# luigifreda/plvs

Hardware: AMD Instinct MI355X
Metric: Mvoxels/sec TSDF integrate (chisel 5 cm / 5 m, 640x480 RGB-D) (higher is better)
Workload: dtype f32; 1 GPU; configs[2] stand-in, STREAMING: see DESIGN.md 4.1 / 4.6; mode=order-free (fixed-point sums; sdf / weight within tolerance), longest_voxel_run=25008, parallelism=chunk-hash shard x1

## Files before the change

### plvs_amd/csrc/tsdf_chisel.hip

```cpp
#include "tsdf_chisel_handle.hpp"
#include "tsdf_chisel_halo.hpp"
#include "tsdf_chisel_ordered.hpp"
#include "tsdf_chisel_order_free.hpp"
#include "tsdf_chisel_carve.hpp"
#include "tsdf_chisel_shard.hpp"
#include "tsdf_chisel_deform.hpp"
#include "tsdf_chisel_scan.hpp"

namespace {

__global__ void pool_init(float* __restrict__ sdf, size_t n) {
  const size_t i = (size_t)blockIdx.x * blockDim.x + threadIdx.x;
  const size_t stride = (size_t)gridDim.x * blockDim.x;
  for (size_t j = i; j < n; j += stride) sdf[j] = 99999.0f;
}

__global__ void selftest_sort_fill(uint32_t* __restrict__ keys, uint32_t* __restrict__ v32, unsigned long long* __restrict__ v64,
                                   uint32_t n, int bits, uint32_t seed) {
  const uint32_t i = blockIdx.x * blockDim.x + threadIdx.x;
  if (i >= n) return;
  uint32_t x = (i + 1u) * 2654435761u + seed;
  x ^= x << 13; x ^= x >> 17; x ^= x << 5;
  x ^= x << 13; x ^= x >> 17; x ^= x << 5;
  keys[i] = bits >= 32 ? x : (x & ((1u << bits) - 1u));
// ... 227 lines not shown
  (void)hipFree(h->weight);
  (void)hipFree(h->kfid);
  (void)hipFree(h->rgbw);
  (void)hipFree(h->d_ctr);
  if (h->h_ctr) (void)hipHostFree(h->h_ctr);
  (void)hipFree(h->d_wctr);
  if (h->h_wctr) (void)hipHostFree(h->h_wctr);
  if (h->h_seq) (void)hipHostFree(h->h_seq);
  if (h->h_offsets) (void)hipHostFree(h->h_offsets);
  (void)hipFree(h->gdir.keys);
  (void)hipFree(h->gdir.slots);
  (void)hipFree(h->miss_keys);
  (void)hipFree(h->miss_ids);
  (void)hipFree(h->miss_count);
  (void)hipFree(h->xdir.keys);
  (void)hipFree(h->xdir.slots);
  (void)hipFree(h->xdir.slot_ids);
  (void)hipFree(h->d_xcount);
  (void)hipFree(h->x_sat);
  if (h->h_sh_counts) (void)hipHostFree(h->h_sh_counts);
  if (h->h_sh_ctl) (void)hipHostFree(h->h_sh_ctl);
  if (h->h_sh_off) (void)hipHostFree(h->h_sh_off);
  h->q_xyz.release(); h->q_rgb.release(); h->q_kfid.release();
  h->w_rec.release(); h->w_seg.release(); h->w_sorted_seg.release(); h->w_chunk_nseg.release();
  h->w_chunk_off.release(); h->w_chunk_fill.release(); h->w_active_off.release(); h->w_masks.release();
  h->w_dummy.release(); h->w_runkey.release(); h->w_run_cnt.release(); h->w_run_off.release(); h->w_val0.release();
  h->w_val1.release(); h->w_seg_cnt.release(); h->w_tile_visits.release(); h->w_deferred.release(); h->w_part_off.release(); h->w_multi_idx.release();
  h->pa_wuu.release(); h->pa_w.release(); h->pa_last.release(); h->pa_cnt.release(); h->pa_done.release();
  h->sh_nrec.release(); h->sh_owner.release(); h->halo_row.release();
  h->sh_ctl.release(); h->sh_seg_reg.release(); h->sh_rec_reg.release(); h->sh_src_off.release(); h->sh_slot_owner.release(); h->sh_run_ctr.release(); h->sh_vkey.release(); h->sh_sat.release(); h->sh_wait.release(); h->sh_run_first.release();
  if (h->ev_fork) (void)hipEventDestroy(h->ev_fork);
  if (h->ev_join) (void)hipEventDestroy(h->ev_join);
  if (h->ev_seg) (void)hipEventDestroy(h->ev_seg);
  if (h->ev_zero) (void)hipEventDestroy(h->ev_zero);
  h->w_rseg.release(); h->w_rpre.release(); h->w_run_matrix.release(); h->w_active_idx.release(); h->w_item_base.release();
  h->w_item_cnt.release(); h->w_item_part0.release(); h->w_part_item.release(); h->w_phist.release();
  h->w_row_heads.release(); h->w_row_tot.release();
  if (h->side) (void)hipStreamDestroy(h->side);
  for (int i = 0; i <= kNumStages; ++i)
    if (h->ev[i]) (void)hipEventDestroy(h->ev[i]);
  h->counts.release();
  h->rec.release(); h->rec_t.release(); h->recc_t.release();
  h->dkey0.release(); h->dkey1.release(); h->didx0.release(); h->didx1.release();
  h->last_pt.release(); h->run_cnt.release(); h->run_dst.release();
  h->tile_first.release(); h->block_first.release(); h->tile_state.release();
  h->heads.release(); h->updated.release(); h->scratch.release(); h->poses.release();
  h->offsets.release(); h->st_xyz.release(); h->st_Twc.release(); h->st_nrm.release(); h->st_rgb.release();
// ... 505 lines not shown
```

### plvs_amd/csrc/tsdf_chisel_handle.hpp

```cpp
#pragma once
#include <vector>

#include "common.hpp"
#include "device_utils.hpp"
#include "tsdf_chisel_core.hpp"
#include "tsdf_directory.hpp"
#include "tsdf_chisel_view.hpp"
#include "tsdf_walk.hpp"
#include "tsdf_walk_plan.hpp"

using namespace plvs;
using namespace plvs::chisel;
using namespace plvs::tsdf;

namespace {

constexpr int kNumStages = 6;
const char* const kStageNames[kNumStages] = {"ray_count", "scan", "ray_tiles", "sort_runs",
                                             "gather_runs", "chain_runs"};
constexpr int kWalkStages = 4;
const char* const kWalkStageNames[kWalkStages] = {"walk_tiles", "sort_segments", "apply_chunks", "fold_colours"};

struct Counters {
  uint32_t total_visits;
// ... 72 lines not shown
  unsigned long long* miss_keys = nullptr;
  int32_t* miss_ids = nullptr;
  uint32_t* miss_count = nullptr;
  uint32_t miss_cap = 0, miss_mask = 0;
  DevBuf<int32_t> offsets;
  DevBuf<float> st_xyz, st_Twc, st_nrm;
  DevBuf<uint8_t> st_rgb;
  DevBuf<uint32_t> st_kfid;
  DevBuf<uint32_t> st_pos, st_scan, st_off;
  plvs_tsdf_stats stats{};
  uint32_t last_updated = 0;
  DevBuf<float> q_xyz;
  DevBuf<uint8_t> q_rgb;
  DevBuf<uint32_t> q_kfid;
  std::vector<int32_t> q_offsets;
  std::vector<float> q_Twc;
  bool q_kfid_given = false;
  WalkCounters* d_wctr = nullptr;
  WalkCounters* h_wctr = nullptr;
  uint32_t* h_seq = nullptr;
  uint32_t seq_next = 0;
  double wait_ema_us[3][3] = {{0.0, 0.0, 0.0}, {0.0, 0.0, 0.0}, {0.0, 0.0, 0.0}};
  DevBuf<uint4> w_rec, w_seg, w_sorted_seg;
  DevBuf<uint4> w_rseg, w_rpre;
  DevBuf<uint32_t> w_run_matrix, w_active_idx, w_item_base, w_item_cnt, w_item_part0, w_part_item, w_phist, w_row_heads, w_row_tot;
  hipEvent_t ev_zero = nullptr;
  hipEvent_t ev_seg = nullptr;
  int last_chain = 0;
  bool last_chain_skipped = false;
  DevBuf<uint32_t> w_chunk_nseg, w_chunk_off, w_chunk_fill, w_active_off, w_masks, w_dummy, w_seg_cnt, w_tile_visits, w_deferred;
  DevBuf<uint32_t> w_part_off, w_multi_idx;
  DevBuf<long long> pa_wuu;
  DevBuf<unsigned long long> pa_w;
  DevBuf<uint32_t> pa_last, pa_cnt, pa_done;
  uint32_t multi_cap = 0;
  uint32_t part_segs = kPartSegs, part_min = kPartMin;
  plvs::tsdf::WalkHistory walk;
  DevBuf<uint32_t> w_runkey, w_run_cnt, w_run_off, w_val0, w_val1;
  int32_t* h_offsets = nullptr;
  size_t h_offsets_cap = 0;
  uint32_t run_r1_log2 = 11;
  float scale_u = 1.f, scale_w = 1.f;
  int stage_set = 0;
  Directory xdir{};
  int32_t* d_xcount = nullptr;
  uint32_t* x_sat = nullptr;
// ... 131 lines not shown
```

### plvs_amd/csrc/tsdf_chisel_order_free.hpp

```cpp
#pragma once
#include "tsdf_chisel_handle.hpp"

namespace {

__global__ void walk_prologue(const float* __restrict__ Twc, int nclouds, Pose* __restrict__ poses,
                              const int32_t* __restrict__ host_offsets, int32_t* __restrict__ offsets,
                              WalkCounters* __restrict__ wctr, Counters* __restrict__ ctr, uint32_t* __restrict__ chunk_nseg,
                              int nseg, int ntile_first = 0) {
  const int i0 = blockIdx.x * blockDim.x + threadIdx.x, stride = gridDim.x * blockDim.x;
  for (int c = i0; c < nclouds; c += stride) make_pose(Twc + 12 * c, &poses[c]);
  for (int c = i0; c < 2 * (nclouds + 1) + ntile_first; c += stride) offsets[c] = host_offsets[c];
  for (int k = i0; k < nseg; k += stride) chunk_nseg[k] = 0u;
  uint32_t* w = reinterpret_cast<uint32_t*>(wctr);
  for (int k = i0; k < (int)(2 * sizeof(WalkCounters) / sizeof(uint32_t)); k += stride) w[k] = 0u;
  if (i0 == 0) {
    ctr->total_visits = 0;
    ctr->err = 0;
    ctr->num_heads = 0;
    ctr->num_updated = 0;
    ctr->max_run = 0;
    ctr->num_desc = 0;
  }
}

// ... 54 lines not shown
  PLVS_HIP_TRY(hipMemset(h->pa_cnt.p, 0, nv * sizeof(uint32_t)));
  PLVS_HIP_TRY(hipMemset(h->pa_done.p, 0, nd * sizeof(uint32_t)));
  h->multi_cap = chunks;
  return PLVS_OK;
}

static int reserve_chunk_tables(plvs_tsdf_chisel* h, size_t chunks, uint32_t part_chunks) {
  PLVS_HIP_TRY(h->w_chunk_nseg.reserve(chunks));
  PLVS_HIP_TRY(h->w_chunk_off.reserve(chunks + 1));
  PLVS_HIP_TRY(h->w_chunk_fill.reserve(chunks));
  PLVS_HIP_TRY(h->w_active_off.reserve(chunks + 1));
  PLVS_HIP_TRY(h->updated.reserve(chunks + 1));
  PLVS_HIP_TRY(h->w_part_off.reserve(chunks + 1));
  PLVS_HIP_TRY(h->w_multi_idx.reserve(chunks + 1));
  return ensure_part_acc(h, part_chunks);
}


struct SegSrc {
  size_t slots;
  uint32_t seg_cap, ntiles;
  const uint32_t* seg_cnt;
};
template <bool kScatter, int kSpan = kSegSpan>
static void launch_seg_pass(plvs_tsdf_chisel* h, const SegSrc& src, hipStream_t q) {
  hipLaunchKernelGGL((seg_pass<kScatter, kSpan>), dim3(ceil_div(src.slots, kSpan)), dim3(256), 0, q, h->w_seg.p, src.seg_cap,
                     src.ntiles, src.seg_cnt, h->w_chunk_nseg.p, h->w_chunk_off.p, h->w_chunk_fill.p, h->w_sorted_seg.p,
                     h->d_wctr);
}

struct SegScan {
  const int32_t* num_chunks;
  int chunk_cap;
  const uint32_t *tile_visits, *run_cnt;
  uint32_t ntiles;
  uint32_t* active_idx;
};
static void launch_seg_scan(plvs_tsdf_chisel* h, const SegScan& a, hipStream_t q) {
  hipLaunchKernelGGL(seg_scan, dim3(1), dim3(1024), 0, q, h->w_chunk_nseg.p, h->w_chunk_off.p, h->w_chunk_fill.p, h->updated.p,
                     h->w_active_off.p, h->d_wctr, a.num_chunks, a.chunk_cap, a.tile_visits, a.run_cnt, a.ntiles,
                     h->w_part_off.p, h->w_multi_idx.p, h->multi_cap, h->part_segs, h->part_min, a.active_idx);
}

static void sort_segments(plvs_tsdf_chisel* h, const SegSrc& src, const SegScan& scan, hipStream_t q) {
  launch_seg_pass<false>(h, src, q);
  launch_seg_scan(h, scan, q);
  launch_seg_pass<true>(h, src, q);
}

template <bool kWide, bool kEmit>
static void launch_apply(plvs_tsdf_chisel* h, const uint4* rec, const uint32_t* d_kfid, const EmitOut& emit, uint32_t last_shift,
// ... 1 lines not shown
  hipLaunchKernelGGL((apply_chunks<kWide, kEmit>), dim3(4096), dim3(kApplyThreads), 0, q, h->w_sorted_seg.p, h->updated.p,
                     h->w_active_off.p, h->w_part_off.p, h->w_multi_idx.p, h->part_segs,
                     PartAcc{h->pa_wuu.p, h->pa_w.p, h->pa_last.p, h->pa_cnt.p, h->pa_done.p}, rec,
                     kEmit ? 0.0 : 1.0 / (double)h->scale_u, kEmit ? 0.0 : 1.0 / (double)h->scale_w, d_kfid,
                     kEmit ? (float*)nullptr : h->sdf, kEmit ? (float*)nullptr : h->weight, kEmit ? (uint32_t*)nullptr : h->kfid,
                     h->d_wctr, emit, last_shift);
}

struct WalkScratch {
  size_t rec_own, seg_own, rec_spill, seg_spill;
};
static WalkScratch walk_scratch(const plvs_tsdf_chisel* h, uint32_t ntiles) {
  WalkScratch w;
  w.rec_own = (size_t)ntiles * kRecStride;
  w.seg_own = (size_t)ntiles * kWalkChunks;
  w.rec_spill = std::max<size_t>(h->w_rec.cap > w.rec_own ? h->w_rec.cap - w.rec_own : 0, (size_t)1 << 16);
  w.seg_spill = std::max<size_t>(h->w_seg.cap / 2 > w.seg_own ? h->w_seg.cap / 2 - w.seg_own : 0, (size_t)1 << 12);
  return w;
}
static int reserve_walk_scratch(plvs_tsdf_chisel* h, uint32_t ntiles, const WalkScratch& w) {
  if (h->w_rec.cap < w.rec_own + w.rec_spill) PLVS_HIP_TRY(h->w_rec.reserve(2 * w.rec_own + w.rec_spill));
  if (h->w_seg.cap < 2 * (w.seg_own + w.seg_spill)) PLVS_HIP_TRY(h->w_seg.reserve(2 * (2 * w.seg_own + w.seg_spill)));
  PLVS_HIP_TRY(h->w_sorted_seg.reserve(h->w_seg.cap));
  const size_t run_slots = (size_t)ntiles << h->run_r1_log2;
  if (h->w_runkey.cap < run_slots) {
    PLVS_HIP_TRY(h->w_runkey.reserve(2 * run_slots));
    PLVS_HIP_TRY(h->w_masks.reserve(2 * run_slots * kMaskWords));
  }
  PLVS_HIP_TRY(h->w_masks.reserve(run_slots * kMaskWords));
  return PLVS_OK;
}
static AccOut walk_out(const plvs_tsdf_chisel* h, const WalkScratch& w, uint32_t* chunk_nseg) {
  return AccOut{h->w_rec.p, (uint32_t)std::min<size_t>(w.rec_own + w.rec_spill, 0xFFFFFFFFu), h->w_seg.p,
                (uint32_t)std::min<size_t>(w.seg_own + w.seg_spill, 0xFFFFFFFFu), h->w_seg_cnt.p, h->w_tile_visits.p, chunk_nseg};
}
static bool grow_walk_scratch(plvs_tsdf_chisel* h, uint32_t ntiles, WalkScratch& w) {
  w.rec_spill = std::max<size_t>(w.rec_spill, (size_t)h->h_wctr->rec_top * 2);
  w.seg_spill = std::max<size_t>(w.seg_spill, (size_t)h->h_wctr->seg_top * 2);
  while ((1u << h->run_r1_log2) < h->h_wctr->run_need) ++h->run_r1_log2;
  return ((size_t)ntiles << h->run_r1_log2) < 0xFFFFFFFFull;
}


struct WalkCall {
  const float* d_xyz;
  const uint8_t* d_rgb;
  const uint32_t* d_kfid;
  int n, nclouds;
  uint32_t ntiles;
  int max_chunks;
  const GridSrc* gsrc;
  const GridSrc* d_grid;
  size_t seg_slots;
  AccOut out;
  RunOut runs;
  const uint32_t* last_count;
  uint32_t collect_seq;
// ... 12 lines not shown
}

static void launch_walk_passes(plvs_tsdf_chisel* h, const WalkPlan& plan, const WalkCall& c, hipStream_t s) {
  for (int i = 0; i < plan.npasses; ++i) {
    const WalkPass& pass = plan.pass[i];
    if (pass.entries == kPlanSmallClass) launch_walk_fast<kFastEntriesSmall>(h, c, pass, s);
    else if (pass.entries == kFastEntries) launch_walk_fast<kFastEntries>(h, c, pass, s);
    else launch_walk_fast<kFastEntriesBig>(h, c, pass, s);
  }
  hipLaunchKernelGGL((walk_tiles<true, true>), dim3(kDeferGrid), dim3(kWalkRays), 0, s, h->P, h->scale_u, h->scale_w, c.d_xyz,
                     c.n, h->offsets.p, c.nclouds, h->poses.p, h->dir, &h->d_ctr->num_chunks, h->d_wctr, h->rgbw,
                     (const uint32_t*)nullptr, c.out, c.runs, TileMap{1u, 0u, 1u}, c.ntiles,
                     (const uint32_t*)(h->w_deferred.p + (size_t)plan.last_list * c.ntiles), c.last_count, kRecStride,
                     plan.pieces, c.d_grid);
}

static int segments_and_apply(plvs_tsdf_chisel* h, const WalkPlan& plan, const WalkCall& c, hipStream_t q) {
  launch_seg_scan(h, SegScan{&h->d_ctr->num_chunks, c.max_chunks, h->w_tile_visits.p, h->w_run_cnt.p, c.ntiles,
                             plan.collect_ready ? h->w_active_idx.p : nullptr}, q);
  if (plan.collect_ready) {
    const bool queued = plan.chain == kChainCollected;
    PLVS_HIP_TRY(hipStreamWaitEvent(q, h->ev_zero, 0));
    hipLaunchKernelGGL(runs_count, dim3(plan.collect_blocks), dim3(kSegSpan), 0, q, h->w_seg.p, h->w_rseg.p, c.ntiles, h->w_seg_cnt.p,
                       h->w_active_idx.p, plan.collect_rows, plan.collect_blocks, h->w_run_matrix.p, h->w_rpre.p, h->d_wctr, c.last_count);
    hipLaunchKernelGGL(runs_rowscan, dim3(std::min<uint32_t>(ceil_div(plan.collect_rows, 4), 1024u)), dim3(256), 0, q,
                       h->w_run_matrix.p, plan.collect_rows, plan.collect_blocks, h->d_wctr, h->w_item_cnt.p);
    hipLaunchKernelGGL(rows_place, dim3(1), dim3(1024), 0, q, h->w_item_cnt.p, plan.collect_rows, plan.collect_bound,
                       (uint32_t)std::min<size_t>(plan.parts_cap, 0xFFFFFFFFu), h->d_wctr,
                       h->w_item_base.p, h->w_item_part0.p, h->w_part_item.p, reinterpret_cast<const uint32_t*>(h->d_ctr),
                       reinterpret_cast<uint32_t*>(h->h_wctr), reinterpret_cast<uint32_t*>(h->h_ctr),
                       (uint32_t)(sizeof(Counters) / sizeof(uint32_t)), queued ? h->h_seq : (uint32_t*)nullptr,
                       queued ? c.collect_seq : 0u);
    PLVS_HIP_TRY(hipEventRecord(h->ev_seg, q));
  }
  const SegSrc src{c.seg_slots, c.out.seg_cap, c.ntiles, h->w_seg_cnt.p};
  if (plan.size_class == 2) launch_seg_pass<true, kSegSpanLong>(h, src, q);
  else launch_seg_pass<true>(h, src, q);
  PLVS_HIP_TRY(stage_mark(h, 2, q));
  launch_apply<false, false>(h, h->w_rec.p, c.d_kfid, EmitOut{}, c.gsrc ? c.gsrc->key_bits : 0u, q);
  PLVS_KERNEL_CHECK();
  PLVS_HIP_TRY(stage_mark(h, 3, q));
  return PLVS_OK;
}

static int launch_fold(plvs_tsdf_chisel* h, const WalkCall& c, uint32_t D, const uint32_t* skeys, const uint32_t* sval,
                       const uint32_t* skip, hipStream_t q) {
  const RunSrc rsrc{h->w_masks.p, (uint32_t)kMaskWords, h->run_r1_log2, TileMap{1u, 0u}, h->offsets.p, c.nclouds,
                    reinterpret_cast<const uint32_t*>(h->offsets.p) + 2 * ((size_t)c.nclouds + 1)};
  const auto kernel = c.gsrc ? fold_colours_masks<true> : fold_colours_masks<false>;
  hipLaunchKernelGGL(kernel, dim3(std::min<size_t>(ceil_div(D, kFoldWaves), 8192)), dim3(64 * kFoldWaves), 0, q, skeys, sval,
                     &h->d_wctr[1].num_desc, rsrc, h->heads.p, c.d_rgb, h->rgbw, &h->d_wctr[1].num_heads, (uint32_t*)nullptr,
                     (uint32_t*)nullptr, skip, c.gsrc ? *c.gsrc : GridSrc{});
  PLVS_KERNEL_CHECK();
  return PLVS_OK;
}

template <int BITS>
static void launch_sort_medium(plvs_tsdf_chisel* h, uint32_t ntiles, int passes, const RunGuard* guard, hipStream_t q) {
  hipLaunchKernelGGL(sort_runs_medium<BITS>, dim3(1), dim3(1024), 0, q, h->w_runkey.p, h->w_run_cnt.p, ntiles, h->run_r1_log2,
                     h->d_wctr + 1, h->dkey0.p, h->w_val0.p, h->dkey1.p, h->w_val1.p, h->w_run_off.p, h->heads.p, passes,
// ... 267 lines not shown
```

### plvs_amd/csrc/tsdf_walk.hpp

```cpp
#pragma once
#include <hip/hip_runtime.h>

#include <cstdint>

#include "tsdf_chisel_core.hpp"
#include "tsdf_directory.hpp"
#include "tsdf_tiles.hpp"
#include "tsdf_walk_table.hpp"

namespace {

using namespace plvs::chisel;
using plvs::tsdf::cloud_of;
using plvs::tsdf::tile_span;
using plvs::tsdf::tile_span_tables;
using plvs::tsdf::TileSpan;
using plvs::tsdf::kCoordBias;
using plvs::tsdf::kErrCoordRange;
using plvs::tsdf::kErrDirectoryMiss;
using plvs::tsdf::kErrPoolFull;
using plvs::tsdf::home_bucket;
using plvs::tsdf::next_bucket;

constexpr int kWalkRays = 512;
// ... 468 lines not shown
__device__ __forceinline__ DirPeek dir_peek(const Directory& d, int cx, int cy, int cz) {
  DirPeek p;
  p.key = kEmptyKey;
  p.slot = -1;
  if (!pack_block(cx, cy, cz, &p.want)) {
    p.want = 0;
    return p;
  }
  const uint32_t h = dir_hash(cx, cy, cz, d.mask);
  p.key = d.keys[h];
  p.slot = d.slots[h];
  return p;
}
__device__ __forceinline__ int dir_peek_slot(const DirPeek& p) { return (p.key == p.want && p.slot >= 0) ? p.slot : -1; }

struct AccOut {
  uint4* rec;
  uint32_t rec_cap;
  uint4* seg;
  uint32_t seg_cap;
  uint32_t* seg_cnt;
  uint32_t* tile_visits;
  uint32_t* chunk_nseg;
};
struct RunOut {
  uint32_t* dkey;
  uint32_t* masks;
  uint32_t* run_cnt;
  uint32_t r1_log2;
  uint4* rseg;
};

constexpr int kMaskCap = kWalkEntries / 4;

__device__ __forceinline__ uint4 pack_suboffsets(const uint32_t* o) {
  return make_uint4(o[0] | (o[1] << 16), o[2] | (o[3] << 16), o[4] | (o[5] << 16), o[6] | (o[7] << 16));
}

struct TileMap {
  uint32_t stride, first;
  uint32_t tables;
  __device__ __host__ uint32_t tile_of(uint32_t local) const { return local * stride + first; }
};

template <bool kAcc, bool kRuns>
__global__ __launch_bounds__(kWalkRays, kWalkEntries > 2048 ? 2 : (kWalkEntries > 1024 ? 4 : 6)) void walk_tiles(
// ... 229 lines not shown
      if (ci[k] >= 0) {
        slot_of[k] = S.cslot[ci[k]];
        if (slot_of[k] >= 0) rank[k] = atomicAdd(&S.ccnt[ci[k] * kSlabs + (int)(vid / kSlabVox)], 1u);
      } else {
        int cx, cy, cz;
        chunk_of_code(chunk_code(ekey[k]), fox, foy, foz, &cx, &cy, &cz);
        slot_of[k] = dir_find_or_insert(dir, cx, cy, cz, num_chunks, &ctr->err);
      }
      if (slot_of[k] >= 0) {
        vkey[k] = (uint32_t)slot_of[k] * (uint32_t)kChunkVox + vid;
        const bool cold = sat ? ((sat[vkey[k] >> 5] >> (vkey[k] & 31u)) & 1u) == 0u : (rgbw[vkey[k]] >> 24) < 254u;
        if (kRuns && cold) {
          need |= 1u << k;
          ++nneed;
          multi = multi || (uint32_t)(ewc[k] >> 32) > 1u;
        }
      }
    }
    const bool any_multi = __syncthreads_or(multi ? 1 : 0) != 0;
    WALK_PROF(5);
    if (kAcc) {
      const bool own_region = flushes == 0;
      uint32_t rbase = tile * rec_stride;
      if (own_region || tid < 64) {
        const int cl = lane;
        uint32_t sub[kSlabs], c = 0;
#pragma unroll
        for (int s = 0; s < kSlabs; ++s) {
          sub[s] = c;
          c += S.ccnt[cl * kSlabs + s];
        }
        uint32_t inc = c, sinc = c ? 1u : 0u;
#pragma unroll
        for (int off = 1; off < 64; off <<= 1) {
          const uint32_t up = (uint32_t)__shfl_up((int)inc, off), sup = (uint32_t)__shfl_up((int)sinc, off);
          if (lane >= off) { inc += up; sinc += sup; }
        }
        const uint32_t tot = (uint32_t)__shfl((int)inc, 63), stot = (uint32_t)__shfl((int)sinc, 63);
        uint32_t sbase = tile * (uint32_t)kWalkChunks;
        if (!own_region) {
          if (tid == 0 && tot) {
            rbase = ntiles * rec_stride + atomicAdd(&ctr->rec_top, tot);
            sbase = ntiles * (uint32_t)kWalkChunks + atomicAdd(&ctr->seg_top, stot);
            if (rbase + tot > out.rec_cap || sbase + stot > out.seg_cap) atomicOr(&ctr->err, kErrScratch);
          }
          rbase = (uint32_t)__shfl((int)rbase, 0);
          sbase = (uint32_t)__shfl((int)sbase, 0);
          if (tid == 0) S.rbase = rbase;
        } else if (tid == 0) {
          out.seg_cnt[tile] = stot;
        }
#pragma unroll
        for (int s = 0; s < kSlabs; ++s) S.cbase[cl * kSlabs + s] = (uint16_t)(inc - c + sub[s]);
        if (c && tid < 64) {
          const uint32_t sg = sbase + sinc - 1u;
          if (sg < out.seg_cap) {
            out.seg[2 * (size_t)sg] = make_uint4((uint32_t)S.cslot[cl], rbase + inc - c, c, gtile);
            out.seg[2 * (size_t)sg + 1] = pack_suboffsets(sub);
            if (out.chunk_nseg) atomicAdd(&out.chunk_nseg[S.cslot[cl]], 1u);
          }
        }
      }
      if (!own_region) {
        __syncthreads();
        rbase = S.rbase;
      }
#pragma unroll
      for (int k = 0; k < kPer; ++k) {
        if (slot_of[k] < 0) continue;
        const int e = tid + k * kWalkRays;
        const uint32_t vid = vkey[k] % (uint32_t)kChunkVox;
        const uint4 r = make_uint4(vid | ((uint32_t)(ewc[k] >> 32) << 12),
                                   grid ? grid_order_key(*grid, gt, elast[k]) : first + elast[k], (uint32_t)e_wuu[e],
                                   (uint32_t)ewc[k]);
        uint32_t at;
        if (ci[k] >= 0) {
          at = rbase + S.cbase[ci[k] * kSlabs + (int)(vid / kSlabVox)] + rank[k];
        } else {
          at = ntiles * rec_stride + atomicAdd(&ctr->rec_top, 1u);
          const uint32_t sg = ntiles * (uint32_t)kWalkChunks + atomicAdd(&ctr->seg_top, 1u);
          if (at >= out.rec_cap || sg >= out.seg_cap) {
            atomicOr(&ctr->err, kErrScratch);
          } else {
            uint32_t sub[kSlabs];
#pragma unroll
            for (int s = 0; s < kSlabs; ++s) sub[s] = (uint32_t)s > vid / kSlabVox ? 1u : 0u;
            out.seg[2 * (size_t)sg] = make_uint4((uint32_t)slot_of[k], at, 1u, gtile);
            out.seg[2 * (size_t)sg + 1] = pack_suboffsets(sub);
            if (out.chunk_nseg) atomicAdd(&out.chunk_nseg[slot_of[k]], 1u);
          }
        }
        if (at < out.rec_cap) out.rec[at] = r;
      }
    }

    ++flushes;
    WALK_PROF(6);
    if (!kRuns) {
      if (single && !was_split) break;
      continue;
    }
    uint32_t inc = nneed;
#pragma unroll
    for (int off = 1; off < 64; off <<= 1) {
      const uint32_t up = (uint32_t)__shfl_up((int)inc, off);
      if (lane >= off) inc += up;
    }
    const uint32_t wave_runs = (uint32_t)__shfl((int)inc, 63);
    if (!any_multi) {
      uint32_t base = 0;
      if (lane == 0 && wave_runs) base = atomicAdd(&S.run_total, wave_runs);
      base = (uint32_t)__shfl((int)base, 0);
      const bool fits_runs = base + wave_runs <= (1u << runs.r1_log2);
      if (!fits_runs && lane == 0) {
        atomicOr(&ctr->err, kErrScratch);
        atomicMax(&ctr->run_need, base + wave_runs);
// ... 267 lines not shown
  WALK_PROF(4);
  if (need) S.any_cold = 1u;
  const bool any_multi = __syncthreads_or(multi ? 1 : 0) != 0;
  const bool any_cold = S.any_cold != 0u;
  WALK_PROF(5);
  const bool too_many = !defer && S.nent > (uint32_t)kLimit;
  if (E == 2048 && tid == 0 && !defer && S.nent > (uint32_t)(kFastEntriesSmall * 7 / 8)) atomicAdd(&ctr->over_small, 1u);
  if (!defer) defer = S.overflow != 0 || too_many;
  if (defer) {
    if (tid == 0) {
      out.seg_cnt[tile] = 0;
      runs.run_cnt[tile] = 0;
      out.tile_visits[tile] = 0;
      deferred[atomicAdd(ndeferred, 1u)] = tile | (too_many ? 0x80000000u : 0u);
    }
    return;
  }
  {
    const uint32_t v = wave_sum(nv);
    if (lane == 0 && v) atomicAdd(&S.vis_total, v);
  }
  const uint32_t rbase = tile * rec_stride;
  uint32_t nruns;
  {
    uint32_t sub[kSlabs], c = 0, rsub[kSlabs], rc = 0;
#pragma unroll
    for (int s = 0; s < kSlabs; ++s) {
      sub[s] = c;
      c += S.ccnt[lane * kSlabs + s];
      rsub[s] = 0;
    }
    uint32_t rinc = 0;
    nruns = 0;
    if (any_cold) {
#pragma unroll
      for (int s = 0; s < kSlabs; ++s) {
        rsub[s] = rc;
        rc += S.rcnt[lane * kSlabs + s];
      }
      rinc = wave_scan_incl(rc);
      nruns = (uint32_t)__builtin_amdgcn_readlane((int)rinc, 63);
#pragma unroll
      for (int s = 0; s < kSlabs; ++s) S.rcbase[lane * kSlabs + s] = (uint16_t)(rinc - rc + rsub[s]);
    }
    const uint32_t both = wave_scan_incl(c | (c ? 1u << 16 : 0u));
    const uint32_t inc = both & 0xFFFFu, sinc = both >> 16;
#pragma unroll
    for (int s = 0; s < kSlabs; ++s) S.cbase[lane * kSlabs + s] = (uint16_t)(inc - c + sub[s]);
    if (wid == 0) {
      const uint32_t stot = (uint32_t)__builtin_amdgcn_readlane((int)sinc, 63);
      if (lane == 0) out.seg_cnt[tile] = stot;
      if (c) {
        const uint32_t sg = tile * (uint32_t)kWalkChunks + sinc - 1u;
        out.seg[2 * (size_t)sg] = make_uint4((uint32_t)S.cslot[lane], rbase + inc - c, c, gtile);
        out.seg[2 * (size_t)sg + 1] = pack_suboffsets(sub);
        if (runs.rseg) {
          runs.rseg[2 * (size_t)sg] = make_uint4((tile << runs.r1_log2) + rinc - rc, rc, 0u, 0u);
          runs.rseg[2 * (size_t)sg + 1] = pack_suboffsets(rsub);
        }
        if (out.chunk_nseg) atomicAdd(&out.chunk_nseg[S.cslot[lane]], 1u);
      }
    }
  }
#pragma unroll
  for (int k = 0; k < kPer; ++k) {
    if (vkey[k] == 0xFFFFFFFFu) continue;
    const uint32_t vid = vkey[k] % (uint32_t)kChunkVox;
    const uint4 r = make_uint4(vid | ((uint32_t)(ewc[k] >> 32) << 12),
                               grid ? grid_order_key(*grid, gt, elast[k]) : first + elast[k],
                               (uint32_t)e_wuu[tid + k * kWalkRays], (uint32_t)ewc[k]);
    out.rec[rbase + S.cbase[ci[k] * kSlabs + (int)(vid / kSlabVox)] + rank[k]] = r;
  }
  WALK_PROF(6);
  const bool fits_runs = nruns <= (1u << runs.r1_log2);
  if (!fits_runs && tid == 0) {
    atomicOr(&ctr->err, kErrScratch);
    atomicMax(&ctr->run_need, nruns);
  }
  uint32_t mrun[kPer];
#pragma unroll
  for (int k = 0; k < kPer; ++k)
    mrun[k] = (need & (1u << k)) ? (uint32_t)S.rcbase[ci[k] * kSlabs + (int)((vkey[k] % (uint32_t)kChunkVox) / kSlabVox)] + rrank[k] : 0xFFFFu;
  if (!any_multi) {
// ... 42 lines not shown
      __syncthreads();
#pragma unroll
      for (int k = 0; k < kPer; ++k) {
        const uint32_t m = (uint32_t)e_midx[tid + k * kWalkRays];
        if (m == 0xFFFFu || m < r0 || m >= r0 + (uint32_t)kMaskCapE) continue;
        const size_t d = ((size_t)tile << runs.r1_log2) + m;
        runs.dkey[d] = vkey[k];
        const uint32_t* mk = raw + (m - r0) * kMaskWords;
        uint4* dst = reinterpret_cast<uint4*>(runs.masks + d * kMaskWords);
#pragma unroll
        for (int q = 0; q < kMaskWords / 4; ++q) dst[q] = make_uint4(mk[4 * q], mk[4 * q + 1], mk[4 * q + 2], mk[4 * q + 3]);
      }
    }
  }
  if (tid == 0) S.run_total = nruns;
  WALK_PROF(7);
  __syncthreads();
  WALK_PROF(8);
  WALK_PROF_END();
  if (tid == 0) {
    runs.run_cnt[tile] = min(S.run_total, 1u << runs.r1_log2);
    out.tile_visits[tile] = S.vis_total;
  }
}

template <int E, bool kGrid = false>
__global__ __launch_bounds__(kWalkRays, walk_fast_waves(E)) void walk_fast(
    Params P, float scale_u, float scale_w, const float* __restrict__ xyz, int npoints,
    const int32_t* __restrict__ offsets, int nclouds, const Pose* __restrict__ poses, Directory dir,
    int32_t* __restrict__ num_chunks, WalkCounters* __restrict__ ctr, const uint32_t* __restrict__ rgbw,
    const uint32_t* __restrict__ sat, AccOut out, RunOut runs, TileMap tmap, uint32_t rec_stride,
    const uint32_t* __restrict__ tile_list, const uint32_t* __restrict__ ntile_list, uint32_t* __restrict__ deferred,
    uint32_t* __restrict__ ndeferred, const GridSrc* __restrict__ grid) {
  if (!tile_list) {
    walk_fast_tile<E, kGrid>(P, scale_u, scale_w, xyz, npoints, offsets, nclouds, poses, dir, num_chunks, ctr, rgbw, sat, out, runs,
                      tmap, rec_stride, deferred, ndeferred, blockIdx.x, false, grid);
    return;
  }
  const uint32_t nlist = *ntile_list;
  for (uint32_t lb = blockIdx.x; lb < nlist; lb += gridDim.x) {
    const uint32_t e = tile_list[lb];
    walk_fast_tile<E, kGrid>(P, scale_u, scale_w, xyz, npoints, offsets, nclouds, poses, dir, num_chunks, ctr, rgbw, sat, out, runs,
                      tmap, rec_stride, deferred, ndeferred, e & 0x7FFFFFFFu, (e >> 31) == 0u, grid);
    __syncthreads();
  }
}

constexpr int kSegSpan = 1024;
constexpr int kSegSpanLong = 4096;
constexpr uint32_t kPartSegs = 256;
constexpr uint32_t kPartMin = 512;
constexpr int kSegTable = 512;
template <bool kScatter, int kSpan = kSegSpan>
__global__ __launch_bounds__(256) void seg_pass(const uint4* __restrict__ seg, uint32_t seg_cap, uint32_t ntiles,
                                                const uint32_t* __restrict__ seg_cnt, uint32_t* __restrict__ chunk_nseg,
                                                const uint32_t* __restrict__ chunk_off, uint32_t* __restrict__ chunk_fill,
                                                uint4* __restrict__ sorted, const WalkCounters* __restrict__ ctr) {
  __shared__ uint32_t hkey[kSegTable], hcnt[kSegTable], hbase[kSegTable];
  const int tid = threadIdx.x;
  const uint32_t own = ntiles * (uint32_t)kWalkChunks;
  const uint32_t n = min(own + ctr->seg_top, seg_cap);
  for (int k = tid; k < kSegTable; k += 256) {
    hkey[k] = 0xFFFFFFFFu;
    hcnt[k] = 0;
  }
  __syncthreads();
  constexpr int kPer = kSpan / 256;
  int ent[kPer];
  uint32_t rnk[kPer], slot[kPer];
#pragma unroll
  for (int q = 0; q < kPer; ++q) {
    const uint32_t j = blockIdx.x * (uint32_t)kSpan + (uint32_t)(q * 256 + tid);
    ent[q] = -2;
    if (j >= n || (j < own && (j % kWalkChunks) >= seg_cnt[j / kWalkChunks])) continue;
    slot[q] = seg[2 * (size_t)j].x;
    uint32_t h = (slot[q] * 2654435761u) >> (32 - 9);
    ent[q] = -1;
    for (int probe = 0; probe < kSegTable; ++probe) {
      uint32_t cur = hkey[h];
      if (cur == 0xFFFFFFFFu) cur = atomicCAS(&hkey[h], 0xFFFFFFFFu, slot[q]);
      if (cur == 0xFFFFFFFFu || cur == slot[q]) {
        ent[q] = (int)h;
        break;
      }
      h = (h + 1) & (kSegTable - 1);
    }
    if (ent[q] >= 0) rnk[q] = atomicAdd(&hcnt[ent[q]], 1u);
  }
  __syncthreads();
  for (int k = tid; k < kSegTable; k += 256) {
    if (hkey[k] == 0xFFFFFFFFu) continue;
    if (kScatter) hbase[k] = chunk_off[hkey[k]] + atomicAdd(&chunk_fill[hkey[k]], hcnt[k]);
    else atomicAdd(&chunk_nseg[hkey[k]], hcnt[k]);
  }
  if (kScatter) __syncthreads();
#pragma unroll
  for (int q = 0; q < kPer; ++q) {
    if (ent[q] == -2) continue;
    const uint32_t j = blockIdx.x * (uint32_t)kSpan + (uint32_t)(q * 256 + tid);
    if (kScatter) {
      const uint32_t at = ent[q] >= 0 ? hbase[ent[q]] + rnk[q] : chunk_off[slot[q]] + atomicAdd(&chunk_fill[slot[q]], 1u);
      sorted[2 * (size_t)at] = seg[2 * (size_t)j];
      sorted[2 * (size_t)at + 1] = seg[2 * (size_t)j + 1];
    } else if (ent[q] == -1) {
      atomicAdd(&chunk_nseg[slot[q]], 1u);
    }
  }
}

__global__ __launch_bounds__(1024) void seg_scan(const uint32_t* __restrict__ chunk_nseg, uint32_t* __restrict__ chunk_off,
                                                 uint32_t* __restrict__ chunk_fill, uint32_t* __restrict__ active,
                                                 uint32_t* __restrict__ active_off, WalkCounters* __restrict__ ctr,
                                                 const int32_t* __restrict__ num_chunks, int max_chunks,
                                                 const uint32_t* __restrict__ tile_visits,
                                                 const uint32_t* __restrict__ run_cnt, uint32_t ntiles,
                                                 uint32_t* __restrict__ part_off, uint32_t* __restrict__ multi_idx,
                                                 uint32_t multi_cap, uint32_t part_segs, uint32_t part_min,
                                                 uint32_t* __restrict__ active_idx = nullptr) {
  __shared__ uint32_t wsum[16], wact[16], wprt[16], wmul[16];
  __shared__ uint32_t carry, acarry, pcarry, mcarry;
  __shared__ unsigned long long vsum[16];
  const int tid = threadIdx.x, lane = tid & 63, wid = tid >> 6;
  const int n = min(*num_chunks, max_chunks);
  if (tid == 0) { carry = 0; acarry = 0; pcarry = 0; mcarry = 0; }
  __syncthreads();
  for (int base = 0; base < n; base += 1024) {
    const int s = base + tid;
    const uint32_t c = s < n ? chunk_nseg[s] : 0u;
    const uint32_t a = c ? 1u : 0u;
    const uint32_t m = c > part_min ? 1u : 0u;
// ... 649 lines not shown
    __syncthreads();
  }
  if (tid == 0) ctr->num_heads = carry;
}

constexpr int kFoldWaves = 4;
constexpr uint32_t kWireRun = 6;
constexpr uint32_t kWireSpans = 6;
constexpr uint32_t kSpanNone = 0xFFFFu;
constexpr uint32_t kWireTileBits = 20;
constexpr uint32_t kCollectPart = 4096;
constexpr int kRunTable = 256;
constexpr int kSpanTiles = kSegSpan / kWalkChunks;
__device__ __forceinline__ uint32_t suboffset_of(const uint4& p, int s) {
  const uint32_t w = s < 2 ? p.x : (s < 4 ? p.y : (s < 6 ? p.z : p.w));
  return (s & 1) ? w >> 16 : w & 0xFFFFu;
}
__device__ __forceinline__ void slab_runs(const uint4& r0, const uint4& r1, int s, uint32_t* first, uint32_t* cnt) {
  const uint32_t lo = suboffset_of(r1, s), hi = s + 1 < kSlabs ? suboffset_of(r1, s + 1) : r0.y;
  *first = r0.x + lo;
  *cnt = hi - lo;
}

__global__ __launch_bounds__(kSegSpan) void runs_count(const uint4* __restrict__ seg, const uint4* __restrict__ rseg, uint32_t ntiles,
                                                       const uint32_t* __restrict__ seg_cnt, const uint32_t* __restrict__ active_idx,
                                                       uint32_t rows_cap, uint32_t nblocks, uint32_t* __restrict__ M,
                                                       uint4* __restrict__ rpre, WalkCounters* __restrict__ ctr,
                                                       const uint32_t* __restrict__ left_to_walk_tiles) {
  __shared__ uint32_t hkey[kRunTable];
  __shared__ alignas(16) uint16_t tbl[kRunTable][kSpanTiles][kSlabs];
  static_assert(kSpanTiles == 16 && kSegSpan == 1024, "16 tiles per block");
  const int tid = threadIdx.x;
  if (*left_to_walk_tiles != 0u || ctr->seg_top != 0u || ctr->err != 0u) {
    if (blockIdx.x == 0 && tid == 0) ctr[1].skip = 1u;
    return;
  }
  static_assert(kRunTable <= kSegSpan && (kRunTable & (kRunTable - 1)) == 0, "a thread per table entry");
  if (tid < kRunTable) hkey[tid] = 0xFFFFFFFFu;
  for (int k = tid; k < kRunTable * kSpanTiles * kSlabs / 2; k += kSegSpan) reinterpret_cast<uint32_t*>(&tbl[0][0][0])[k] = 0u;
  __syncthreads();
  const uint32_t j = blockIdx.x * (uint32_t)kSegSpan + (uint32_t)tid;
  const uint32_t tile = j / kWalkChunks;
  const int tl = tid / kWalkChunks;
  int ent = -1;
  if (tile < ntiles && (j % kWalkChunks) < seg_cnt[tile]) {
    const uint4 r0 = rseg[2 * (size_t)j], r1 = rseg[2 * (size_t)j + 1];
    const uint32_t slot = seg[2 * (size_t)j].x;
    if (r0.y != 0u) {
      uint32_t h = (slot * 2654435761u) >> (32 - log2_of(kRunTable));
      for (int probe = 0; probe < kRunTable; ++probe) {
        uint32_t cur = hkey[h];
        if (cur == 0xFFFFFFFFu) cur = atomicCAS(&hkey[h], 0xFFFFFFFFu, slot);
        if (cur == 0xFFFFFFFFu || cur == slot) {
          ent = (int)h;
          break;
        }
        h = (h + 1) & (kRunTable - 1);
      }
      if (ent < 0) {
        ctr[1].skip = 1u;
      } else {
        uint32_t c[kSlabs];
#pragma unroll
        for (int s = 0; s < kSlabs; ++s) {
          uint32_t f;
          slab_runs(r0, r1, s, &f, &c[s]);
        }
        *reinterpret_cast<uint4*>(&tbl[ent][tl][0]) = pack_suboffsets(c);
// ... 664 lines not shown
```

Baseline: 83750 Mvoxels/s.

## Assign segment tickets during walk and place segments without a scatter pass

The walk kernels now keep the per-chunk position returned by the chunk_nseg atomicAdd and save it to a new seg_ticket buffer. A new seg_place kernel, or the runs_count kernel when the collect path is ready, writes each segment straight to chunk_off plus its ticket. This replaces the hashed seg_pass scatter kernel and drops its long-span variant. The cost is one extra per-segment ticket buffer with its writes, and the placement work is merged into runs_count ahead of that kernel's early-exit check.

```diff
diff --git a/plvs_amd/csrc/tsdf_chisel.hip b/plvs_amd/csrc/tsdf_chisel.hip
--- a/plvs_amd/csrc/tsdf_chisel.hip
+++ b/plvs_amd/csrc/tsdf_chisel.hip
@@ -273,7 +273,7 @@
   if (h->h_sh_ctl) (void)hipHostFree(h->h_sh_ctl);
   if (h->h_sh_off) (void)hipHostFree(h->h_sh_off);
   h->q_xyz.release(); h->q_rgb.release(); h->q_kfid.release();
-  h->w_rec.release(); h->w_seg.release(); h->w_sorted_seg.release(); h->w_chunk_nseg.release();
+  h->w_rec.release(); h->w_seg.release(); h->w_sorted_seg.release(); h->w_seg_ticket.release(); h->w_chunk_nseg.release();
   h->w_chunk_off.release(); h->w_chunk_fill.release(); h->w_active_off.release(); h->w_masks.release();
   h->w_dummy.release(); h->w_runkey.release(); h->w_run_cnt.release(); h->w_run_off.release(); h->w_val0.release();
   h->w_val1.release(); h->w_seg_cnt.release(); h->w_tile_visits.release(); h->w_deferred.release(); h->w_part_off.release(); h->w_multi_idx.release();
diff --git a/plvs_amd/csrc/tsdf_chisel_handle.hpp b/plvs_amd/csrc/tsdf_chisel_handle.hpp
--- a/plvs_amd/csrc/tsdf_chisel_handle.hpp
+++ b/plvs_amd/csrc/tsdf_chisel_handle.hpp
@@ -118,6 +118,7 @@
   uint32_t seq_next = 0;
   double wait_ema_us[3][3] = {{0.0, 0.0, 0.0}, {0.0, 0.0, 0.0}, {0.0, 0.0, 0.0}};
   DevBuf<uint4> w_rec, w_seg, w_sorted_seg;
+  DevBuf<uint32_t> w_seg_ticket;
   DevBuf<uint4> w_rseg, w_rpre;
   DevBuf<uint32_t> w_run_matrix, w_active_idx, w_item_base, w_item_cnt, w_item_part0, w_part_item, w_phist, w_row_heads, w_row_tot;
   hipEvent_t ev_zero = nullptr;
diff --git a/plvs_amd/csrc/tsdf_chisel_order_free.hpp b/plvs_amd/csrc/tsdf_chisel_order_free.hpp
--- a/plvs_amd/csrc/tsdf_chisel_order_free.hpp
+++ b/plvs_amd/csrc/tsdf_chisel_order_free.hpp
@@ -100,11 +100,20 @@
   uint32_t seg_cap, ntiles;
   const uint32_t* seg_cnt;
 };
-template <bool kScatter, int kSpan = kSegSpan>
+template <bool kScatter>
 static void launch_seg_pass(plvs_tsdf_chisel* h, const SegSrc& src, hipStream_t q) {
-  hipLaunchKernelGGL((seg_pass<kScatter, kSpan>), dim3(ceil_div(src.slots, kSpan)), dim3(256), 0, q, h->w_seg.p, src.seg_cap,
+  hipLaunchKernelGGL((seg_pass<kScatter>), dim3(ceil_div(src.slots, kSegSpan)), dim3(256), 0, q, h->w_seg.p, src.seg_cap,
                      src.ntiles, src.seg_cnt, h->w_chunk_nseg.p, h->w_chunk_off.p, h->w_chunk_fill.p, h->w_sorted_seg.p,
                      h->d_wctr);
+}
+static SegPlace seg_place_args(const plvs_tsdf_chisel* h, uint32_t seg_cap) {
+  return SegPlace{h->w_seg_ticket.p, h->w_chunk_off.p, h->w_sorted_seg.p, (uint32_t)std::min<size_t>(h->w_sorted_seg.cap / 2, 0xFFFFFFFFu),
+                  seg_cap};
+}
+static void launch_seg_place(plvs_tsdf_chisel* h, const SegSrc& src, hipStream_t q) {
+  const SegPlace a = seg_place_args(h, src.seg_cap);
+  hipLaunchKernelGGL(seg_place, dim3(ceil_div(src.slots, 256)), dim3(256), 0, q, h->w_seg.p, a.ticket, src.seg_cap, src.ntiles,
+                     src.seg_cnt, a.chunk_off, a.sorted, a.sorted_cap, h->d_wctr);
 }
 
 struct SegScan {
@@ -152,6 +161,7 @@
   if (h->w_rec.cap < w.rec_own + w.rec_spill) PLVS_HIP_TRY(h->w_rec.reserve(2 * w.rec_own + w.rec_spill));
   if (h->w_seg.cap < 2 * (w.seg_own + w.seg_spill)) PLVS_HIP_TRY(h->w_seg.reserve(2 * (2 * w.seg_own + w.seg_spill)));
   PLVS_HIP_TRY(h->w_sorted_seg.reserve(h->w_seg.cap));
+  PLVS_HIP_TRY(h->w_seg_ticket.reserve(h->w_seg.cap / 2));
   const size_t run_slots = (size_t)ntiles << h->run_r1_log2;
   if (h->w_runkey.cap < run_slots) {
     PLVS_HIP_TRY(h->w_runkey.reserve(2 * run_slots));
@@ -162,7 +172,8 @@
 }
 static AccOut walk_out(const plvs_tsdf_chisel* h, const WalkScratch& w, uint32_t* chunk_nseg) {
   return AccOut{h->w_rec.p, (uint32_t)std::min<size_t>(w.rec_own + w.rec_spill, 0xFFFFFFFFu), h->w_seg.p,
-                (uint32_t)std::min<size_t>(w.seg_own + w.seg_spill, 0xFFFFFFFFu), h->w_seg_cnt.p, h->w_tile_visits.p, chunk_nseg};
+                (uint32_t)std::min<size_t>(w.seg_own + w.seg_spill, 0xFFFFFFFFu), h->w_seg_cnt.p, h->w_tile_visits.p, chunk_nseg,
+                chunk_nseg ? h->w_seg_ticket.p : nullptr};
 }
 static bool grow_walk_scratch(plvs_tsdf_chisel* h, uint32_t ntiles, WalkScratch& w) {
   w.rec_spill = std::max<size_t>(w.rec_spill, (size_t)h->h_wctr->rec_top * 2);
@@ -221,7 +232,8 @@
     const bool queued = plan.chain == kChainCollected;
     PLVS_HIP_TRY(hipStreamWaitEvent(q, h->ev_zero, 0));
     hipLaunchKernelGGL(runs_count, dim3(plan.collect_blocks), dim3(kSegSpan), 0, q, h->w_seg.p, h->w_rseg.p, c.ntiles, h->w_seg_cnt.p,
-                       h->w_active_idx.p, plan.collect_rows, plan.collect_blocks, h->w_run_matrix.p, h->w_rpre.p, h->d_wctr, c.last_count);
+                       h->w_active_idx.p, plan.collect_rows, plan.collect_blocks, h->w_run_matrix.p, h->w_rpre.p, h->d_wctr, c.last_count,
+                       seg_place_args(h, c.out.seg_cap));
     hipLaunchKernelGGL(runs_rowscan, dim3(std::min<uint32_t>(ceil_div(plan.collect_rows, 4), 1024u)), dim3(256), 0, q,
                        h->w_run_matrix.p, plan.collect_rows, plan.collect_blocks, h->d_wctr, h->w_item_cnt.p);
     hipLaunchKernelGGL(rows_place, dim3(1), dim3(1024), 0, q, h->w_item_cnt.p, plan.collect_rows, plan.collect_bound,
@@ -232,9 +244,7 @@
                        queued ? c.collect_seq : 0u);
     PLVS_HIP_TRY(hipEventRecord(h->ev_seg, q));
   }
-  const SegSrc src{c.seg_slots, c.out.seg_cap, c.ntiles, h->w_seg_cnt.p};
-  if (plan.size_class == 2) launch_seg_pass<true, kSegSpanLong>(h, src, q);
-  else launch_seg_pass<true>(h, src, q);
+  if (!plan.collect_ready) launch_seg_place(h, SegSrc{c.seg_slots, c.out.seg_cap, c.ntiles, h->w_seg_cnt.p}, q);
   PLVS_HIP_TRY(stage_mark(h, 2, q));
   launch_apply<false, false>(h, h->w_rec.p, c.d_kfid, EmitOut{}, c.gsrc ? c.gsrc->key_bits : 0u, q);
   PLVS_KERNEL_CHECK();
diff --git a/plvs_amd/csrc/tsdf_walk.hpp b/plvs_amd/csrc/tsdf_walk.hpp
--- a/plvs_amd/csrc/tsdf_walk.hpp
+++ b/plvs_amd/csrc/tsdf_walk.hpp
@@ -514,6 +514,7 @@
   uint32_t* seg_cnt;
   uint32_t* tile_visits;
   uint32_t* chunk_nseg;
+  uint32_t* seg_ticket;
 };
 struct RunOut {
   uint32_t* dkey;
@@ -789,6 +790,7 @@
     if (kAcc) {
       const bool own_region = flushes == 0;
       uint32_t rbase = tile * rec_stride;
+      uint32_t ticket = 0, ticket_sg = 0xFFFFFFFFu;
       if (own_region || tid < 64) {
         const int cl = lane;
         uint32_t sub[kSlabs], c = 0;
@@ -822,9 +824,12 @@
         if (c && tid < 64) {
           const uint32_t sg = sbase + sinc - 1u;
           if (sg < out.seg_cap) {
+            if (out.chunk_nseg) {
+              ticket = atomicAdd(&out.chunk_nseg[S.cslot[cl]], 1u);
+              ticket_sg = sg;
+            }
             out.seg[2 * (size_t)sg] = make_uint4((uint32_t)S.cslot[cl], rbase + inc - c, c, gtile);
             out.seg[2 * (size_t)sg + 1] = pack_suboffsets(sub);
-            if (out.chunk_nseg) atomicAdd(&out.chunk_nseg[S.cslot[cl]], 1u);
           }
         }
       }
@@ -840,7 +845,7 @@
         const uint4 r = make_uint4(vid | ((uint32_t)(ewc[k] >> 32) << 12),
                                    grid ? grid_order_key(*grid, gt, elast[k]) : first + elast[k], (uint32_t)e_wuu[e],
                                    (uint32_t)ewc[k]);
-        uint32_t at;
+        uint32_t at, own_ticket = 0, own_sg = 0xFFFFFFFFu;
         if (ci[k] >= 0) {
           at = rbase + S.cbase[ci[k] * kSlabs + (int)(vid / kSlabVox)] + rank[k];
         } else {
@@ -854,11 +859,16 @@
             for (int s = 0; s < kSlabs; ++s) sub[s] = (uint32_t)s > vid / kSlabVox ? 1u : 0u;
             out.seg[2 * (size_t)sg] = make_uint4((uint32_t)slot_of[k], at, 1u, gtile);
             out.seg[2 * (size_t)sg + 1] = pack_suboffsets(sub);
-            if (out.chunk_nseg) atomicAdd(&out.chunk_nseg[slot_of[k]], 1u);
+            if (out.chunk_nseg) {
+              own_ticket = atomicAdd(&out.chunk_nseg[slot_of[k]], 1u);
+              own_sg = sg;
+            }
           }
         }
         if (at < out.rec_cap) out.rec[at] = r;
-      }
+        if (own_sg != 0xFFFFFFFFu) out.seg_ticket[own_sg] = own_ticket;
+      }
+      if (ticket_sg != 0xFFFFFFFFu) out.seg_ticket[ticket_sg] = ticket;
     }
 
     ++flushes;
@@ -1172,6 +1182,7 @@
   }
   const uint32_t rbase = tile * rec_stride;
   uint32_t nruns;
+  uint32_t ticket = 0, ticket_sg = 0xFFFFFFFFu;
   {
     uint32_t sub[kSlabs], c = 0, rsub[kSlabs], rc = 0;
 #pragma unroll
@@ -1202,13 +1213,16 @@
       if (lane == 0) out.seg_cnt[tile] = stot;
       if (c) {
         const uint32_t sg = tile * (uint32_t)kWalkChunks + sinc - 1u;
+        if (out.chunk_nseg) {
+          ticket = atomicAdd(&out.chunk_nseg[S.cslot[lane]], 1u);
+          ticket_sg = sg;
+        }
         out.seg[2 * (size_t)sg] = make_uint4((uint32_t)S.cslot[lane], rbase + inc - c, c, gtile);
         out.seg[2 * (size_t)sg + 1] = pack_suboffsets(sub);
         if (runs.rseg) {
           runs.rseg[2 * (size_t)sg] = make_uint4((tile << runs.r1_log2) + rinc - rc, rc, 0u, 0u);
           runs.rseg[2 * (size_t)sg + 1] = pack_suboffsets(rsub);
         }
-        if (out.chunk_nseg) atomicAdd(&out.chunk_nseg[S.cslot[lane]], 1u);
       }
     }
   }
@@ -1297,6 +1311,7 @@
     runs.run_cnt[tile] = min(S.run_total, 1u << runs.r1_log2);
     out.tile_visits[tile] = S.vis_total;
   }
+  if (ticket_sg != 0xFFFFFFFFu) out.seg_ticket[ticket_sg] = ticket;
 }
 
 template <int E, bool kGrid = false>
@@ -1322,11 +1337,10 @@
 }
 
 constexpr int kSegSpan = 1024;
-constexpr int kSegSpanLong = 4096;
 constexpr uint32_t kPartSegs = 256;
 constexpr uint32_t kPartMin = 512;
 constexpr int kSegTable = 512;
-template <bool kScatter, int kSpan = kSegSpan>
+template <bool kScatter>
 __global__ __launch_bounds__(256) void seg_pass(const uint4* __restrict__ seg, uint32_t seg_cap, uint32_t ntiles,
                                                 const uint32_t* __restrict__ seg_cnt, uint32_t* __restrict__ chunk_nseg,
                                                 const uint32_t* __restrict__ chunk_off, uint32_t* __restrict__ chunk_fill,
@@ -1340,7 +1354,7 @@
     hcnt[k] = 0;
   }
   __syncthreads();
-  constexpr int kPer = kSpan / 256;
+  constexpr int kSpan = kSegSpan, kPer = kSpan / 256;
   int ent[kPer];
   uint32_t rnk[kPer], slot[kPer];
 #pragma unroll
@@ -1381,6 +1395,30 @@
       atomicAdd(&chunk_nseg[slot[q]], 1u);
     }
   }
+}
+
+__device__ __forceinline__ bool segment_written(uint32_t j, uint32_t seg_cap, uint32_t ntiles, const uint32_t* __restrict__ seg_cnt,
+                                                const WalkCounters* __restrict__ ctr) {
+  const uint32_t own = ntiles * (uint32_t)kWalkChunks;
+  if (j < own) return (j % kWalkChunks) < seg_cnt[j / kWalkChunks];
+  return j < min(own + ctr->seg_top, seg_cap);
+}
+__device__ __forceinline__ void place_segment(const uint4* __restrict__ seg, const uint32_t* __restrict__ seg_ticket,
+                                              const uint32_t* __restrict__ chunk_off, uint4* __restrict__ sorted,
+                                              uint32_t sorted_cap, uint32_t j) {
+  const uint4 d0 = seg[2 * (size_t)j], d1 = seg[2 * (size_t)j + 1];
+  const uint32_t at = chunk_off[d0.x] + seg_ticket[j];
+  if (at >= sorted_cap) return;
+  sorted[2 * (size_t)at] = d0;
+  sorted[2 * (size_t)at + 1] = d1;
+}
+__global__ __launch_bounds__(256) void seg_place(const uint4* __restrict__ seg, const uint32_t* __restrict__ seg_ticket,
+                                                 uint32_t seg_cap, uint32_t ntiles, const uint32_t* __restrict__ seg_cnt,
+                                                 const uint32_t* __restrict__ chunk_off, uint4* __restrict__ sorted,
+                                                 uint32_t sorted_cap, const WalkCounters* __restrict__ ctr) {
+  if (ctr->err != 0u) return;
+  const uint32_t j = blockIdx.x * 256u + threadIdx.x;
+  if (segment_written(j, seg_cap, ntiles, seg_cnt, ctr)) place_segment(seg, seg_ticket, chunk_off, sorted, sorted_cap, j);
 }
 
 __global__ __launch_bounds__(1024) void seg_scan(const uint32_t* __restrict__ chunk_nseg, uint32_t* __restrict__ chunk_off,
@@ -2076,15 +2114,29 @@
   *cnt = hi - lo;
 }
 
+struct SegPlace {
+  const uint32_t *ticket, *chunk_off;
+  uint4* sorted;
+  uint32_t sorted_cap, seg_cap;
+};
 __global__ __launch_bounds__(kSegSpan) void runs_count(const uint4* __restrict__ seg, const uint4* __restrict__ rseg, uint32_t ntiles,
                                                        const uint32_t* __restrict__ seg_cnt, const uint32_t* __restrict__ active_idx,
                                                        uint32_t rows_cap, uint32_t nblocks, uint32_t* __restrict__ M,
                                                        uint4* __restrict__ rpre, WalkCounters* __restrict__ ctr,
-                                                       const uint32_t* __restrict__ left_to_walk_tiles) {
+                                                       const uint32_t* __restrict__ left_to_walk_tiles, SegPlace place) {
   __shared__ uint32_t hkey[kRunTable];
   __shared__ alignas(16) uint16_t tbl[kRunTable][kSpanTiles][kSlabs];
   static_assert(kSpanTiles == 16 && kSegSpan == 1024, "16 tiles per block");
   const int tid = threadIdx.x;
+  const uint32_t j = blockIdx.x * (uint32_t)kSegSpan + (uint32_t)tid;
+  const uint32_t tile = j / kWalkChunks;
+  const bool written = tile < ntiles && (j % kWalkChunks) < seg_cnt[tile];
+  if (ctr->err == 0u) {
+    if (written) place_segment(seg, place.ticket, place.chunk_off, place.sorted, place.sorted_cap, j);
+    const uint32_t own = ntiles * (uint32_t)kWalkChunks, n = min(own + ctr->seg_top, place.seg_cap);
+    for (uint32_t k = own + j; k < n; k += gridDim.x * (uint32_t)kSegSpan)
+      place_segment(seg, place.ticket, place.chunk_off, place.sorted, place.sorted_cap, k);
+  }
   if (*left_to_walk_tiles != 0u || ctr->seg_top != 0u || ctr->err != 0u) {
     if (blockIdx.x == 0 && tid == 0) ctr[1].skip = 1u;
     return;
@@ -2093,11 +2145,9 @@
   if (tid < kRunTable) hkey[tid] = 0xFFFFFFFFu;
   for (int k = tid; k < kRunTable * kSpanTiles * kSlabs / 2; k += kSegSpan) reinterpret_cast<uint32_t*>(&tbl[0][0][0])[k] = 0u;
   __syncthreads();
-  const uint32_t j = blockIdx.x * (uint32_t)kSegSpan + (uint32_t)tid;
-  const uint32_t tile = j / kWalkChunks;
   const int tl = tid / kWalkChunks;
   int ent = -1;
-  if (tile < ntiles && (j % kWalkChunks) < seg_cnt[tile]) {
+  if (written) {
     const uint4 r0 = rseg[2 * (size_t)j], r1 = rseg[2 * (size_t)j + 1];
     const uint32_t slot = seg[2 * (size_t)j].x;
     if (r0.y != 0u) {
```

Measured after the change: 87580 Mvoxels/s (median of 6 runs). 4.6% higher.
